# peteroh23/ModulationDetectionCNN

Measured on AMD Instinct MI355X. Metric: I/Q frames/sec (2x128, VT-CNN2, batch=2^20), higher is better.
Workload: dtype bf16; 1 GPU; vtcnn2-c11-bf16-n2^20; topology=vtcnn2, classes=11, frames_per_gpu=1048576, global_batch=1048576, parallelism=batch-shard x1 (no collective), outputs=softmax probabilities f32 + argmax int32, frames_per_forward_call=1048576, full=False

## Files before the change

### modulationdetectioncnn_amd/csrc/mdc_internal.h

```cpp
#pragma once
#include <hip/hip_runtime.h>
#include <cstdarg>
#include <cstdint>
#include <cstdio>
#include <exception>
#include <mutex>
#include <new>
#include <string>
#include <type_traits>
#include <vector>

#include "mdc.h"

namespace mdc {

void set_error(const char* fmt, ...);

template <class Fn>
inline int guarded(const char* what, Fn&& fn) noexcept {
    try {
        return fn();
    } catch (const std::bad_alloc&) {
        set_error("%s: out of host memory", what);
        return MDC_ENOMEM;
// ... 17 lines not shown

constexpr int kRows = 2;
constexpr int kSamples = 128;
constexpr int kFrameFloats = kRows * kSamples;

constexpr int kC1 = 256;
constexpr int kW1 = 130;
constexpr int kC2 = 80;
constexpr int kW2 = 132;
constexpr int kFeat = kC2 * kW2;
constexpr int kHid = 256;

__host__ __device__ constexpr int feat16_index(int w, int o) {
    return (w >> 1) * (2 * kC2) + (o < 64 ? (w & 1) * 64 + o : 128 + 2 * (o - 64) + (w & 1));
}

__host__ __device__ constexpr int feat8_index(int w, int o) {
    return (w >> 2) * (4 * kC2) + (o < 64 ? ((w >> 1) & 1) * 128 + 8 * (o >> 2) + 4 * (w & 1) + (o & 3) : 256 + 4 * (o - 64) + (w & 3));
}

__device__ __forceinline__ uint2 load8_unaligned(const unsigned char* p) {
    uint2 r;
    __builtin_memcpy(&r, p, 8);
    return r;
}

struct NfArgs {
    unsigned char* flags;
    unsigned long long* count;
    int poison;
// ... 148 lines not shown
```

### modulationdetectioncnn_amd/csrc/vtcnn2.hip

```cpp
#include "dense_chain_common.h"

#include <algorithm>
#include <cmath>

namespace mdc {

namespace {

__device__ __forceinline__ void glds16(const void* g, void* lds_wave_base) {
    const unsigned l = (unsigned)(size_t)(__attribute__((address_space(3))) unsigned char*)lds_wave_base;
    asm volatile("global_load_lds_dwordx4 %0, off" ::"v"(g), "{m0}"(l) : "memory");
}
__device__ __forceinline__ void glds_drain_and_barrier() {
    asm volatile("s_waitcnt vmcnt(0)" ::: "memory");
    __syncthreads();
}

constexpr int kChunk = 16;
constexpr int kNChunk = kC1 / kChunk;
constexpr int kWChunkFloats = 2 * 3 * 5 * 4 * 64;
constexpr int kXld = 133;
constexpr int kXinFloats = 4 * 2 * 16 * kXld;
constexpr size_t kConvF32Lds = (2 * kWChunkFloats + kXinFloats) * sizeof(float);

// ... 345 lines not shown
#pragma unroll
    for (int r = 0; r < 4; ++r) {
        const long row = row0 + fq * 4 + r;
        if (row < n) hid[row * kHid + col] = fmaxf(acc[r] + bias, 0.f);
    }
}

template <typename T>
__global__ void vt_unpermute_kernel(const T* __restrict__ feat, long n, float* __restrict__ out, float unscale) {
    const long i = (long)blockIdx.x * blockDim.x + threadIdx.x;
    if (i >= n * kFeat) return;
    const long f = i / kFeat;
    const int r = (int)(i % kFeat);
    const int o = r / kW2, w = r % kW2;
    if constexpr (sizeof(T) == 2) {
        const T v = feat[f * kFeat + feat16_index(w, o)];
        out[i] = __uint_as_float(((unsigned)v) << 16) * unscale;
    } else {
        out[i] = feat[(f * kW2 + w) * kC2 + o];
    }
}

__global__ void vt_unpermute8_kernel(const unsigned char* __restrict__ feat, long n, float* __restrict__ out, float unscale) {
    const long i = (long)blockIdx.x * blockDim.x + threadIdx.x;
    if (i >= n * kFeat) return;
    const long f = i / kFeat;
    const int r = (int)(i % kFeat);
    const int o = r / kW2, w = r % kW2;
    const unsigned v = feat[f * kFeat + feat8_index(w, o)];
    const int e = (int)((v >> 3) & 15u), mant = (int)(v & 7u);
    float mag = e == 0 ? ldexpf((float)mant, -9) : ldexpf(1.f + (float)mant * 0.125f, e - 7);
// ... 181 lines not shown
```

### modulationdetectioncnn_amd/csrc/vtcnn2_bf16.hip

```cpp
#include "vtcnn2_bf16_common.h"
#include "vtcnn2_sched_common.h"

#include <cmath>

#include <cstdlib>
#include <cstring>
#include <type_traits>

namespace mdc {

namespace {

#ifdef MDC_ALTERNATES
__global__ __launch_bounds__(256, 1) void vt_conv_bf16_kernel(const float* __restrict__ x, long n,
                                                              const u32x4* __restrict__ wq,
                                                              const u32x2* __restrict__ a1q,
                                                              const float* __restrict__ b2,
                                                              unsigned short* __restrict__ feat) {
    extern __shared__ __attribute__((aligned(16))) unsigned char smem[];
    unsigned* img = reinterpret_cast<unsigned*>(smem);
    float* part = reinterpret_cast<float*>(smem + (size_t)2 * kImgWords * 4);
    const int tid = threadIdx.x, lane = tid & 63;
    const int q = __builtin_amdgcn_readfirstlane(tid >> 6);
    const int nl = lane & 15, g = lane >> 4;
// ... 18 lines not shown

    for (int i = tid; i < 2 * kImgWords; i += 256) img[i] = ((i & 63) >= 48) ? 0x3F803F80u : 0u;
    __syncthreads();

    const long ngroups = (n + 15) >> 4;
    long grp = blockIdx.x;
    if (grp < ngroups)
        for (int k = 0; k < 4; ++k) stage_quarter(k, x, n, grp * 16, img, tid);
    __syncthreads();

    int buf = 0;
    for (; grp < ngroups; grp += gridDim.x, buf ^= 1) {
        const unsigned* im = img + buf * kImgWords + lane;
        const long frame0 = grp * 16;
        const long fme = frame0 + nl;
        unsigned short* fbase = feat + fme * (long)(kW2 * kC2) + 4 * g;
        const long gnext = grp + gridDim.x;

        f32x4 acc[3][5];
#pragma unroll
        for (int a = 0; a < 3; ++a)
#pragma unroll
            for (int b = 0; b < 5; ++b) acc[a][b] = f32x4{0.f, 0.f, 0.f, 0.f};
        bf16x8 Bf[2][2][2];
        f32x4 X[4][2];
        f32x4 rp[4];
        float rc[4];
        using I0 = std::integral_constant<int, 0>;
        using I1 = std::integral_constant<int, 1>;
        using I2 = std::integral_constant<int, 2>;

// ... 50 lines not shown
            const float* pw = part + PB * kPartFloats;
#pragma unroll
            for (int k = 0; k < 4; ++k) {
                rp[k] = *reinterpret_cast<const f32x4*>(pw + ((k * 5 + q) * 64 + lane) * 4);
                rc[k] = pw[((k * 5 + 4) * 64 + lane) * 4 + q];
            }
        };
        auto red_finish = [&](int w) {
            const f32x4 s = (rp[0] + rp[1]) + (rp[2] + rp[3]);
            u32x2 o;
            const f32x4 bq = *reinterpret_cast<const f32x4*>(bq_lds);
            o[0] = pack2relu(s[0] + bq[0], s[1] + bq[1]);
            o[1] = pack2relu(s[2] + bq[2], s[3] + bq[3]);
            const float t = ((rc[0] + rc[1]) + (rc[2] + rc[3])) + *b4_lds;
            const unsigned short t16 = (unsigned short)pack2relu(t, 0.f);
            unsigned short* frow = fbase - 4 * g;
            *reinterpret_cast<u32x2*>(frow + feat16_index(w, 16 * q + 4 * g)) = o;
            frow[feat16_index(w, 64 + 4 * g + q)] = t16;
        };
#define MDC_SB() __builtin_amdgcn_sched_barrier(0)
        auto step = [&](int v, auto par_next, auto first_tag, auto last_tag, f32x4 (&a0)[5], f32x4 (&a1)[5], f32x4 (&a2)[5]) {
            constexpr bool FIRST = decltype(first_tag)::value != 0, LAST = decltype(last_tag)::value != 0;
            using PB = std::integral_constant<int, 1 - decltype(par_next)::value>;
            if (!FIRST) { x_fence(I1{}); pack(PB{}, I1{}, I0{}); pack(PB{}, I1{}, I1{}); }
            if (!LAST) conv1_load(v + 1, par_next, I0{});
            tap(PB{}, I2{}, I0{}, I0{}, a2, false); tap(PB{}, I2{}, I0{}, I1{}, a2, false);
            tap(PB{}, I2{}, I1{}, I0{}, a2, false); tap(PB{}, I2{}, I1{}, I1{}, a2, false);
            part_write(PB{}, a2);
            if (!LAST) { conv1(par_next, I0{}); conv1_load(v + 1, par_next, I1{}); }
            tap(PB{}, I1{}, I0{}, I0{}, a1, false); tap(PB{}, I1{}, I0{}, I1{}, a1, false);
            tap(PB{}, I1{}, I1{}, I0{}, a1, false);
            if (!LAST) { x_fence(I0{}); pack(par_next, I0{}, I0{}); pack(par_next, I0{}, I1{}); }
            tap(PB{}, I1{}, I1{}, I1{}, a1, false);
// ... 129 lines not shown
```

### modulationdetectioncnn_amd/csrc/vtcnn2_bf16_dense1.hip

```cpp
#include "vtcnn2_bf16_common.h"
#include "dense_chain_common.h"

#include <cstdlib>

namespace mdc {

namespace {

constexpr int kBM = 256, kBN = 256, kBK = 64;
constexpr int kTileBytes = kBM * kBK * 2;
constexpr size_t kDenseBf16Lds = (size_t)4 * kTileBytes;
constexpr size_t kDenseHeadLds = (size_t)128 * kChainXld * 4;
static_assert(kDenseHeadLds >= kDenseBf16Lds, "the fused-head form allocates the larger of the two");
constexpr int kNT = kFeat / kBK;

__device__ __forceinline__ bf16x8 cvt_e4m3x8(u32x2 r) {
    const bf16x2 p0 = __builtin_amdgcn_cvt_scalef32_pk_bf16_fp8(r[0], 1.0f, false);
    const bf16x2 p1 = __builtin_amdgcn_cvt_scalef32_pk_bf16_fp8(r[0], 1.0f, true);
    const bf16x2 p2 = __builtin_amdgcn_cvt_scalef32_pk_bf16_fp8(r[1], 1.0f, false);
    const bf16x2 p3 = __builtin_amdgcn_cvt_scalef32_pk_bf16_fp8(r[1], 1.0f, true);
    return bf16x8{p0[0], p0[1], p1[0], p1[1], p2[0], p2[1], p3[0], p3[1]};
}


#if defined(MDC_ALTERNATES) || defined(MDC_ABLATIONS)
template <int ABL>
__global__ __launch_bounds__(512) void vt_dense1_bf16_kernel(const unsigned short* __restrict__ feat, long n,
                                                             const unsigned short* __restrict__ w1t,
                                                             const float* __restrict__ c1,
// ... 1 lines not shown
    extern __shared__ __attribute__((aligned(16))) unsigned char smem[];
    const int tid = threadIdx.x, lane = tid & 63;
    const int wv = __builtin_amdgcn_readfirstlane(tid >> 6);
    const int wr = wv >> 2, wc = wv & 3;
    const int fr = lane & 15, fg = lane >> 4;
    const long row0 = (long)blockIdx.x * kBM;

    const int srow = lane >> 3, spos = lane & 7;
    const unsigned short* asrc[4];
    const unsigned short* bsrc[4];
#pragma unroll
    for (int p = 0; p < 4; ++p) {
        const int r = (wv * 4 + p) * 8 + srow;
        long gr = (ABL == 1 ? 0 : row0) + r;
        if (gr >= n) gr = n - 1;
        asrc[p] = feat + gr * (long)kFeat + ((spos ^ (r & 7)) * 8);
        bsrc[p] = w1t + r * kBK + ((spos ^ (r & 7)) * 8);
    }
    auto stage = [&](int t, int b) {
        if (ABL == 3 && t > 1) return;
        unsigned char* A = smem + (size_t)b * 2 * kTileBytes;
        unsigned char* B = A + kTileBytes;
#pragma unroll
        for (int p = 0; p < 4; ++p) {
            glds16(asrc[p] + t * kBK, A + (wv * 4 + p) * 1024);
            glds16(bsrc[p] + (long)t * (kBN * kBK), B + (wv * 4 + p) * 1024);
        }
    };

    f32x4 acc[8][4];
#pragma unroll
    for (int i = 0; i < 8; ++i)
#pragma unroll
        for (int j = 0; j < 4; ++j) acc[i][j] = f32x4{0.f, 0.f, 0.f, 0.f};

    auto compute = [&](int b) {
        const unsigned char* A = smem + (size_t)b * 2 * kTileBytes;
        const unsigned char* B = A + kTileBytes;
#pragma unroll
        for (int ks = 0; ks < 2; ++ks) {
// ... 114 lines not shown
    const int wr = wv >> 2, wc = wv & 3;
    const int fr = lane & 15, fg = lane >> 4;
    const long row0 = (long)blockIdx.x * kBM;

    const int srow = lane >> 3, spos = lane & 7;
    const unsigned short* src[4][2];
#pragma unroll
    for (int j = 0; j < 2; ++j) {
        const int u = (wv * 2 + j) * 8 + srow;
        const int sw = (spos ^ (u & 7)) * 8;
        const int arow_lo = 128 * (u >> 6) + (u & 63);
        const int brow_lo = 64 * (u >> 5) + (u & 31);
        long g0 = (ABL == 1 ? 0 : row0) + arow_lo, g3 = (ABL == 1 ? 0 : row0) + arow_lo + 64;
        if (g0 >= n) g0 = n - 1;
        if (g3 >= n) g3 = n - 1;
        src[0][j] = feat + g0 * (long)kFeat + sw;
        src[3][j] = feat + g3 * (long)kFeat + sw;
        src[1][j] = w1t + brow_lo * kBK + sw;
        src[2][j] = w1t + (brow_lo + 32) * kBK + sw;
    }
    const unsigned char* src8[2] = {nullptr, nullptr};
    if constexpr (F8) {
        const int u = wv * 16 + (lane >> 2);
        const int sw = ((lane & 3) ^ ((u >> 2) & 3)) * 16;
        const int arow_lo = 128 * (u >> 6) + (u & 63);
        long g0 = row0 + arow_lo, g3 = row0 + arow_lo + 64;
        if (g0 >= n) g0 = n - 1;
        if (g3 >= n) g3 = n - 1;
        const unsigned char* f8 = reinterpret_cast<const unsigned char*>(feat);
        src8[0] = f8 + g0 * (long)kFeat + sw;
        src8[1] = f8 + g3 * (long)kFeat + sw;
    }
    auto stage_unit = [&](int t, int unit, int b) {
        if (ABL == 2 && (unit == 1 || unit == 2) && (t & 1)) return;
        unsigned char* dst = smem + ((size_t)b * 4 + unit) * kUnitBytes + (wv * 2) * 1024;
        if constexpr (F8) {
            if (unit == 0 || unit == 3) {
                glds16(src8[unit == 3] + (long)t * kBK, smem + ((size_t)b * 4 + unit) * kUnitBytes + wv * 1024);
                return;
            }
        }
        if (unit == 0 || unit == 3) {
            glds16_nt(src[unit][0] + (long)t * kBK, dst);
            glds16_nt(src[unit][1] + (long)t * kBK, dst + 1024);
        } else {
            glds16(src[unit][0] + (long)t * (kBN * kBK), dst);
            glds16(src[unit][1] + (long)t * (kBN * kBK), dst + 1024);
        }
    };

    auto frag = [&](const unsigned char* unit_base, int u, int ks) {
        return *reinterpret_cast<const bf16x8*>(unit_base + u * 128 + (((ks * 4 + fg) ^ (u & 7)) * 16));
    };

    f32x4 acc[8][4];
#pragma unroll
    for (int i = 0; i < 8; ++i)
#pragma unroll
        for (int j = 0; j < 4; ++j) acc[i][j] = f32x4{0.f, 0.f, 0.f, 0.f};
// ... 138 lines not shown

    d1_epilogue<HEAD>(acc, smem, row0, n, lane, wv, c1, hid, w2pack, n_out, probs, labels);
}


template <bool F8>
__global__ __launch_bounds__(64) void vt_dense1_bf16_small_kernel(const unsigned short* __restrict__ feat, long n,
                                                                  const unsigned short* __restrict__ w1t,
                                                                  const float* __restrict__ c1, float* __restrict__ hid) {
    const int lane = threadIdx.x, fr = lane & 15, fg = lane >> 4;
    const long row0 = (long)blockIdx.x * 16;
    const int col0 = blockIdx.y * 16;
    long ar = row0 + fr;
    if (ar >= n) ar = n - 1;
    using AFrag = typename std::conditional<F8, u32x2, bf16x8>::type;
    const unsigned char* ap = reinterpret_cast<const unsigned char*>(feat) + (ar * (long)kFeat + fg * 8) * (F8 ? 1 : 2);
    const unsigned short* bp = w1t + (long)(col0 + fr) * kBK + fg * 8;
    f32x4 acc = f32x4{0.f, 0.f, 0.f, 0.f};
    constexpr int kU = 5, kBlocks = kNT / kU;
    static_assert(kNT % kU == 0 && kBlocks % 2 == 1, "blocks: an even count in the loop, the last one drained after it");
    AFrag a0[kU][2], a1[kU][2];
    bf16x8 b0[kU][2], b1[kU][2];
    auto load = [&](AFrag (&af)[kU][2], bf16x8 (&bfr)[kU][2], int blk) {
#pragma unroll
        for (int u = 0; u < kU; ++u)
#pragma unroll
            for (int ks = 0; ks < 2; ++ks) {
                af[u][ks] = *reinterpret_cast<const AFrag*>(ap + ((blk * kU + u) * kBK + ks * 32) * (F8 ? 1 : 2));
                bfr[u][ks] = *reinterpret_cast<const bf16x8*>(bp + (long)(blk * kU + u) * (kBN * kBK) + ks * 32);
            }
    };
    auto mma = [&](const AFrag (&af)[kU][2], const bf16x8 (&bfr)[kU][2]) {
#pragma unroll
        for (int u = 0; u < kU; ++u)
#pragma unroll
            for (int ks = 0; ks < 2; ++ks) {
                bf16x8 a;
                if constexpr (F8) a = cvt_e4m3x8(af[u][ks]); else a = af[u][ks];
                acc = __builtin_amdgcn_mfma_f32_16x16x32_bf16(a, bfr[u][ks], acc, 0, 0, 0);
            }
    };
    load(a0, b0, 0);
    for (int blk = 0; blk < kBlocks - 1; blk += 2) {
// ... 19 lines not shown
template <bool F8>
__global__ __launch_bounds__(256) void vt_dense1_bf16_coop_kernel(const unsigned short* __restrict__ feat, long n,
                                                                  const unsigned short* __restrict__ w1t,
                                                                  const float* __restrict__ c1, float* __restrict__ hid) {
    extern __shared__ __attribute__((aligned(16))) unsigned char smem[];
    const int tid = threadIdx.x, lane = tid & 63, fr = lane & 15, fg = lane >> 4;
    const int wv = __builtin_amdgcn_readfirstlane(tid >> 6);
    const long row0 = (long)blockIdx.x * 16;
    const int col0 = blockIdx.y * 16;
    long ar = row0 + fr;
    if (ar >= n) ar = n - 1;
    const unsigned char* src;
    long kstep;
    if (wv < 2) {
        if constexpr (F8) { src = reinterpret_cast<const unsigned char*>(feat) + ar * (long)kFeat + fg * 16; kstep = kBK; }
        else { src = reinterpret_cast<const unsigned char*>(feat + ar * (long)kFeat + fg * 8 + (wv & 1) * 32); kstep = 2L * kBK; }
    } else {
        src = reinterpret_cast<const unsigned char*>(w1t + (long)(col0 + fr) * kBK + fg * 8 + (wv & 1) * 32);
        kstep = 2L * kBN * kBK;
    }
    const bool copies = !(F8 && wv == 1);
    static_assert(kRing % kGrp == 0, "groups do not straddle the ring's end");
    constexpr int kAhead = kRing / kGrp - 1;
    constexpr int kGroups = kNT / kGrp, kTail = kNT - kGroups * kGrp;
    auto issue = [&](int g) {
#pragma unroll
        for (int j = 0; j < kGrp; ++j) {
            const int t = g * kGrp + j, tc = t < kNT ? t : kNT - 1;
            if (copies) glds16_async(src + tc * kstep, smem + (size_t)(t % kRing) * 4096 + wv * 1024);
        }
    };
// ... 144 lines not shown
```

### modulationdetectioncnn_amd/csrc/vtcnn2_bf16_sched.hip

```cpp
#include "vtcnn2_bf16_common.h"
#include "vtcnn2_sched_common.h"

#include <cmath>
#include <cstdlib>
#include <type_traits>

namespace mdc {

namespace {

constexpr int kNV = 24;

struct SchedState {
    u32x4 Wv[kNV];
    u32x4 Wa[kWFrags - kNV];
    f32x4 bias[5];
    u32x4 A1[2];
    unsigned Bf[2][2][2][4];
    f32x16 X[2];
    f32x4 rp[4];
    float rc[4];
    float tprev;
    u32x4 L0[3];
    u32x4 L1;
// ... 14 lines not shown
        static_assert(IDX >= kNV, "padded form written for the AGPR-resident fragments only");
        asm volatile("s_nop 1\n\tv_mfma_f32_16x16x32_bf16 %0, %1, %2, %0" : "+a"(acc[OT]) : "a"(st.Wa[IDX - kNV]), "v"(b));
    } else {
        if constexpr (IDX < kNV) asm volatile("v_mfma_f32_16x16x32_bf16 %0, %1, %2, %0" : "+a"(acc[OT]) : "v"(st.Wv[IDX]), "v"(b));
        else asm volatile("v_mfma_f32_16x16x32_bf16 %0, %1, %2, %0" : "+a"(acc[OT]) : "a"(st.Wa[IDX - kNV]), "v"(b));
    }
}
template <int SP, int U>
__device__ __forceinline__ void sch_packop(SchedState& st) {
    constexpr int CT = U >> 3, j = U & 7;
    unsigned& d = st.Bf[SP][CT][j >> 2][j & 3];
    const float lo = st.X[CT][2 * j], hi = st.X[CT][2 * j + 1];
    asm volatile("v_cvt_pk_bf16_f32 %0, %1, %2 clamp" : "=v"(d) : "v"(lo), "v"(hi));
}
template <int V12, bool FIRST, bool LAST, int ABL, bool RANGE = false>
__device__ __forceinline__ void sch_step(SchedState& st, int v, int q, unsigned short* fbase, f32x4 (&acc)[3][5], int wlo = 0) {
    constexpr int PAR = V12 & 1, PN = 1 - PAR;
    constexpr int R1 = (V12 + 1) & 3, S0 = ((V12 + 1) >> 2) % 3, SN = (S0 + 1) % 3;
    constexpr bool kLoadEven = (V12 & 3) == 1 && !LAST, kLoadOdd = (V12 & 3) == 3 && !LAST;
    constexpr int LSLOT = ((V12 >> 2) + 1) % 3;
    constexpr bool kExch = ABL != 2 && ABL != 6, kFin = ABL != 3 && ABL != 6, kC1 = ABL != 5 && ABL != 6;
    f32x4 (&a2)[5] = acc[V12 % 3];
    f32x4 (&a1)[5] = acc[(V12 + 1) % 3];
    f32x4 (&a0)[5] = acc[(V12 + 2) % 3];
    const unsigned load_addr = st.im_addr + ((v >> 2) * 16 + (kLoadEven ? 16 : 24));
    FinTmp ft;
    FinOut fo;
    constexpr int OP = (V12 + 1) & 1;
#define FIN(K) do { if (!FIRST && kFin) sch_fin_clamp<K, OP>(st, ft, fo); } while (0)
#define PREP(I) do { if (!LAST && kC1 && ABL != 11) sch_prep<R1, S0, SN, I>(st); } while (0)
#define C1M(CT) do { if (!LAST && kC1) sch_conv1_mfma<R1, S0, CT>(st); } while (0)
#define ST(W) do { if (!FIRST && kFin && (W == 0 || OP == 1)) { if (ABL == 7) { if (W == 0) asm volatile("" ::"v"(fo.o0), "v"(fo.o1)); else asm volatile("" ::"v"(fo.tt)); } else if (!RANGE || v - 1 >= wlo) sch_store<W>(fo, fbase, v - 1, q, st.gs); } } while (0)
#define WR(OT) do { if (kExch && ABL != 8) sch_part_write<PAR, OT>(st, a2[OT]); } while (0)
#define PK(N) do { if (!LAST && kC1 && ABL != 10) sch_packop<PN, N>(st); } while (0)
#define RD(R) do { if (kExch && ABL != 9) sch_red_load1<PAR, R>(st); } while (0)
#define LD() do { if (kC1 && ABL != 11) { if (kLoadEven) sch_load_even<LSLOT>(st, load_addr); else if (kLoadOdd) sch_load_odd(st, load_addr); } } while (0)
#ifdef MDC_F8_PROBE_HALF_BARRIER
    constexpr bool kHalfBarrierSkip = (V12 & 1) == 1;
#else
    constexpr bool kHalfBarrierSkip = false;
#endif
#define HANDOFF() do { \
        if (ABL == 1 || kHalfBarrierSkip) asm volatile("s_waitcnt lgkmcnt(0)" ::: "memory"); \
        else if (kExch) asm volatile("s_waitcnt lgkmcnt(0)\n\ts_barrier" ::: "memory"); \
        asm volatile("" ::"a"(a2[0]), "a"(a2[1]), "a"(a2[2]), "a"(a2[3]), "a"(a2[4])); } while (0)
    sch_wait_lds(st);
    sch_tap<PAR, 2, 0, RANGE && (V12 == 1 || V12 == 2)>(st, a2); FIN(0);
// ... 47 lines not shown
    sch_tap<PAR, 0, 6>(st, a0); HANDOFF();
    sch_tap<PAR, 0, 7>(st, a0); RD(0);
    sch_tap<PAR, 0, 8>(st, a0); RD(1);
    sch_tap<PAR, 0, 9>(st, a0); RD(2);
    sch_tap<PAR, 0, 10>(st, a0); RD(3);
    sch_tap<PAR, 0, 11>(st, a0); RD(4);
    sch_tap<PAR, 0, 12>(st, a0); RD(5);
    sch_tap<PAR, 0, 13>(st, a0); RD(6);
    sch_tap<PAR, 0, 14>(st, a0); RD(7);
    sch_tap<PAR, 0, 15>(st, a0); LD();
    sch_tap<PAR, 0, 16>(st, a0);
    sch_tap<PAR, 0, 17>(st, a0);
    sch_tap<PAR, 0, 18>(st, a0);
    sch_tap<PAR, 0, 19>(st, a0);
    if (ABL == 10 && !LAST) asm volatile("" ::"v"(st.X[0]), "v"(st.X[1]));
#undef FIN
#undef PREP
#undef C1M
#undef ST
#undef WR
#undef PK
#undef RD
#undef LD
#undef HANDOFF
}

template <int ABL, bool U8 = false, bool RANGE = false>
__global__ __launch_bounds__(256, 1) void vt_conv_bf16_sched_kernel(const float* __restrict__ x, long n,
                                                                    const u32x4* __restrict__ wq, const u32x4* __restrict__ a1q,
                                                                    const float* __restrict__ b2, unsigned short* __restrict__ feat,
// ... 37 lines not shown

    for (int i = tid; i < 2 * kSImgWords; i += 256) img[i] = ((((i / kS) & 63) >= 32) && ((i % kS) & 1)) ? 0x3F803F80u : 0u;
    __syncthreads();
    const long ngroups = (n + 15) >> 4;
    long grp = blockIdx.x;
    if (grp < ngroups)
        for (int k = 0; k < 4; ++k) sch_stage_write(k, stage_decode<U8>(stage_load<U8>(k, x, n, grp * 16, tid, hop2), tid, scale), n, grp * 16, img, tid);
    __syncthreads();
    const int rng = RANGE ? (int)blockIdx.y : 0;
    const int S = 12 * rng;
    const int wlo = rng ? S + 2 : 0;

    int buf = 0;
    for (; grp < ngroups; grp += gridDim.x, buf ^= 1) {
        st.im_addr = img_lds + (buf * kSImgWords + lane * kS) * 4;
        unsigned short* fbase = feat + (grp * 16 + fs) * (long)(kW2 * kC2);
        const long gnext = RANGE ? ngroups : grp + gridDim.x;
        f32x4 acc[3][5];
        {
            const u32x4 zero = u32x4{0u, 0u, 0u, 0u};
#pragma unroll
            for (int b = 0; b < 5; ++b) {
                asm volatile("s_nop 1\n\tv_mfma_f32_16x16x32_bf16 %0, %1, %1, %2" : "=&a"(acc[0][b]) : "v"(zero), "a"(st.bias[b]));
                asm volatile("v_mfma_f32_16x16x32_bf16 %0, %1, %1, %2" : "=&a"(acc[1][b]) : "v"(zero), "a"(st.bias[b]));
            }
        }

        sch_load_even<0>(st, st.im_addr + (S >> 2) * 16);
        sch_load_odd(st, st.im_addr + (S >> 2) * 16 + 8);
        sch_wait_lds(st);
        sch_conv1_mfma<0, 0, 0>(st); sch_conv1_mfma<0, 0, 1>(st);
        asm volatile("s_nop 7\n\ts_nop 7\n\ts_nop 7\n\ts_nop 7\n\ts_nop 7\n\ts_nop 7\n\ts_nop 7\n\ts_nop 7" : "+v"(st.X[0]), "+v"(st.X[1]));
        [&]<int... N>(std::integer_sequence<int, N...>) { (sch_packop<0, N>(st), ...); }(std::make_integer_sequence<int, 16>{});
        asm volatile("s_nop 1");

        sch_step<0, true, false, ABL, RANGE>(st, S, q, fbase, acc, wlo);
        const int iters = RANGE ? (rng < 10 ? 1 : 0) : 10;
        int v = S + 1;
        typename StageRaw<U8>::type sv{};
        for (int it = 0; it < iters; ++it, v += 12) {
            if constexpr (!RANGE) {
                if (it >= 6 && gnext < ngroups) sch_stage_write(it - 6, stage_decode<U8>(sv, tid, scale), n, gnext * 16, img + (buf ^ 1) * kSImgWords, tid);
                if (it >= 5 && it < 9 && gnext < ngroups) sv = stage_load<U8>(it - 5, x, n, gnext * 16, tid, hop2);
            }
            sch_step<1, false, false, ABL, RANGE>(st, v + 0, q, fbase, acc, wlo);
            sch_step<2, false, false, ABL, RANGE>(st, v + 1, q, fbase, acc, wlo);
            sch_step<3, false, false, ABL, RANGE>(st, v + 2, q, fbase, acc, wlo);
            sch_step<4, false, false, ABL, RANGE>(st, v + 3, q, fbase, acc, wlo);
            sch_step<5, false, false, ABL, RANGE>(st, v + 4, q, fbase, acc, wlo);
            sch_step<6, false, false, ABL, RANGE>(st, v + 5, q, fbase, acc, wlo);
            sch_step<7, false, false, ABL, RANGE>(st, v + 6, q, fbase, acc, wlo);
            sch_step<8, false, false, ABL, RANGE>(st, v + 7, q, fbase, acc, wlo);
            sch_step<9, false, false, ABL, RANGE>(st, v + 8, q, fbase, acc, wlo);
            sch_step<10, false, false, ABL, RANGE>(st, v + 9, q, fbase, acc, wlo);
            sch_step<11, false, false, ABL, RANGE>(st, v + 10, q, fbase, acc, wlo);
            sch_step<0, false, false, ABL, RANGE>(st, v + 11, q, fbase, acc, wlo);
        }
        const int vt = RANGE ? v : 121;
        sch_step<1, false, false, ABL, RANGE>(st, vt, q, fbase, acc, wlo);
        if constexpr (RANGE) {
            if (rng < 10) {
                FinOut fo;
                sch_wait_lds(st);
                sch_fin_all_clamp<1>(st, fo);
                sch_store<0>(fo, fbase, vt, q, st.gs);
                sch_store<1>(fo, fbase, vt, q, st.gs);
                asm volatile("s_nop 7\n\ts_nop 7" ::"a"(acc[0][0]), "a"(acc[1][0]), "a"(acc[2][0]));
                __syncthreads();
                continue;
            }
        }
        sch_step<2, false, false, ABL, RANGE>(st, 122, q, fbase, acc, wlo);
        sch_step<3, false, false, ABL, RANGE>(st, 123, q, fbase, acc, wlo);
        sch_step<4, false, false, ABL, RANGE>(st, 124, q, fbase, acc, wlo);
        sch_step<5, false, false, ABL, RANGE>(st, 125, q, fbase, acc, wlo);
        sch_step<6, false, false, ABL, RANGE>(st, 126, q, fbase, acc, wlo);
        sch_step<7, false, false, ABL, RANGE>(st, 127, q, fbase, acc, wlo);
        sch_step<8, false, false, ABL, RANGE>(st, 128, q, fbase, acc, wlo);
        sch_step<9, false, true, ABL, RANGE>(st, 129, q, fbase, acc, wlo);
        auto finish_store = [&](auto odd, int w) {
            FinOut fo;
            sch_wait_lds(st);
            sch_fin_all_clamp<decltype(odd)::value>(st, fo);
            sch_store<0>(fo, fbase, w, q, st.gs);
            if constexpr (decltype(odd)::value) sch_store<1>(fo, fbase, w, q, st.gs);
        };
        using Even = std::integral_constant<int, 0>;
        using Odd = std::integral_constant<int, 1>;
        finish_store(Odd{}, 129);
        asm volatile("s_nop 7\n\ts_nop 7");
        sch_part_write<0, 0>(st, acc[1][0]); sch_part_write<0, 1>(st, acc[1][1]); sch_part_write<0, 2>(st, acc[1][2]);
        sch_part_write<0, 3>(st, acc[1][3]); sch_part_write<0, 4>(st, acc[1][4]);
        asm volatile("s_waitcnt lgkmcnt(0)\n\ts_barrier" ::: "memory");
        sch_red_load<0>(st);
        asm volatile("" ::"a"(acc[1][0]), "a"(acc[1][1]), "a"(acc[1][2]), "a"(acc[1][3]), "a"(acc[1][4]));
        finish_store(Even{}, 130);
        sch_part_write<1, 0>(st, acc[2][0]); sch_part_write<1, 1>(st, acc[2][1]); sch_part_write<1, 2>(st, acc[2][2]);
        sch_part_write<1, 3>(st, acc[2][3]); sch_part_write<1, 4>(st, acc[2][4]);
        asm volatile("s_waitcnt lgkmcnt(0)\n\ts_barrier" ::: "memory");
        sch_red_load<1>(st);
        asm volatile("" ::"a"(acc[2][0]), "a"(acc[2][1]), "a"(acc[2][2]), "a"(acc[2][3]), "a"(acc[2][4]));
        finish_store(Odd{}, 131);
        __syncthreads();
    }
}

}

int vtcnn2_bf16_pack_sched(mdc_model* m) {
    const float* k1 = m->hk[0].data();
    const float* b1 = m->hb[0].data();
    const float* k2 = m->hk[1].data();
    int rc;
    std::vector<unsigned short> wq((size_t)4 * kWFrags * 64 * 8);
    for (int q = 0; q < 4; ++q)
        for (int ct = 0; ct < 2; ++ct)
            for (int j = 0; j < 3; ++j)
// ... 68 lines not shown
```

### modulationdetectioncnn_amd/csrc/vtcnn2_fp8_conv.hip

```cpp
#include "vtcnn2_bf16_common.h"
#include "vtcnn2_sched_common.h"

#include <cmath>
#include <cstdlib>

namespace mdc {

namespace {

using u32x8 = __attribute__((ext_vector_type(8))) unsigned;
constexpr int kF8Frags = 15;
constexpr int kF8NV = 7;

struct Fp8State {
    u32x8 Wv[kF8NV];
    u32x8 Wa[kF8Frags - kF8NV];
    f32x4 bias[5];
    u32x4 A1[2];
    unsigned Bf[2][8];
    unsigned one;
    unsigned scb;
    float sc9;
    f32x16 X[2];
    unsigned T[16];
// ... 200 lines not shown

    for (int i = tid; i < 2 * kSImgWords; i += 256) img[i] = ((((i / kS) & 63) >= 32) && ((i % kS) & 1)) ? 0x3F803F80u : 0u;
    __syncthreads();
    const long ngroups = (n + 15) >> 4;
    long grp = blockIdx.x;
    if (grp < ngroups)
        for (int k = 0; k < 4; ++k) sch_stage_write(k, stage_decode<U8>(stage_load<U8>(k, x, n, grp * 16, tid, hop2), tid, scale), n, grp * 16, img, tid);
    __syncthreads();
    const int rng = RANGE ? (int)blockIdx.y : 0;
    const int S = 12 * rng;
    const int wlo = rng ? S + 2 : 0;

    int buf = 0;
    for (; grp < ngroups; grp += gridDim.x, buf ^= 1) {
        st.im_addr = img_lds + (buf * kSImgWords + lane * kS) * 4;
        FeatT* fbase = feat + (grp * 16 + fs) * (long)(kW2 * kC2);
        const long gnext = RANGE ? ngroups : grp + gridDim.x;
        f32x4 acc[3][5];
        {
            const u32x4 zero = u32x4{0u, 0u, 0u, 0u};
#pragma unroll
            for (int b = 0; b < 5; ++b) {
                asm volatile("s_nop 1\n\tv_mfma_f32_16x16x32_bf16 %0, %1, %1, %2" : "=&a"(acc[0][b]) : "v"(zero), "a"(st.bias[b]));
                asm volatile("v_mfma_f32_16x16x32_bf16 %0, %1, %1, %2" : "=&a"(acc[1][b]) : "v"(zero), "a"(st.bias[b]));
            }
        }
        sch_load_even<0>(st, st.im_addr + (S >> 2) * 16);
        sch_load_odd(st, st.im_addr + (S >> 2) * 16 + 8);
        sch_wait_lds(st);
        sch_conv1_mfma<0, 0, 0>(st); sch_conv1_mfma<0, 0, 1>(st);
        asm volatile("s_nop 7\n\ts_nop 7\n\ts_nop 7\n\ts_nop 7\n\ts_nop 7\n\ts_nop 7\n\ts_nop 7\n\ts_nop 7" : "+v"(st.X[0]), "+v"(st.X[1]));
// ... 225 lines not shown
```

### modulationdetectioncnn_amd/csrc/vtcnn2_sched_common.h

```cpp
#pragma once
#include "vtcnn2_bf16_common.h"

#include <type_traits>
#include <utility>

namespace mdc {

namespace {

constexpr int kS = 140;
constexpr int kSImgWords = 64 * kS;
constexpr long kConvRangeFrames = 1024;
constexpr size_t kSchedLds = (size_t)2 * kSImgWords * 4 + (size_t)2 * kPartFloats * 4;

using f32x16 = __attribute__((ext_vector_type(16))) float;

template <int SLOT, class S>
__device__ __forceinline__ void sch_load_even(S& st, unsigned entry_addr) {
    asm volatile("ds_read_b128 %0, %1" : "=v"(st.L0[SLOT]) : "v"(entry_addr) : "memory");
}
template <class S>
__device__ __forceinline__ void sch_load_odd(S& st, unsigned entry_addr) {
    asm volatile("ds_read2_b64 %0, %1 offset0:0 offset1:1" : "=v"(st.L1) : "v"(entry_addr) : "memory");
}
// ... 51 lines not shown
    else if constexpr (K == 14) asm volatile("v_add_f32 %0, %1, %2" : "=v"(f.a) : "v"(st.rc[0]), "v"(st.rc[1]));
    else if constexpr (K == 15) asm volatile("v_add_f32 %0, %1, %2" : "=v"(f.b) : "v"(st.rc[2]), "v"(st.rc[3]));
    else if constexpr (K == 16) {
        if constexpr (ODD) asm volatile("v_add_f32 %0, %1, %2" : "=v"(f.t) : "v"(f.a), "v"(f.b));
        else asm volatile("v_add_f32 %0, %1, %2" : "=v"(st.tprev) : "v"(f.a), "v"(f.b));
    } else if constexpr (ODD) asm volatile("v_cvt_pk_bf16_f32 %0, %1, %2 clamp" : "=v"(out.tt) : "v"(st.tprev), "v"(f.t));
}
template <int ODD, class S>
__device__ __forceinline__ void sch_fin_all_clamp(S& st, FinOut& out) {
    FinTmp f;
    [&]<int... K>(std::integer_sequence<int, K...>) { (sch_fin_clamp<K, ODD>(st, f, out), ...); }(std::make_integer_sequence<int, 18>{});
}

template <int WHICH>
__device__ __forceinline__ void sch_store(const FinOut& fo, unsigned short* frow, int w, int q, int gs) {
    unsigned short* pair = frow + (long)(w >> 1) * (2 * kC2);
    if constexpr (WHICH == 0) *reinterpret_cast<u32x2*>(pair + (w & 1) * 64 + 16 * q + 4 * gs) = u32x2{fo.o0, fo.o1};
    else *reinterpret_cast<unsigned*>(pair + 128 + 2 * (4 * q + gs)) = fo.tt;
}

__device__ __forceinline__ void sch_stage_write(int k, float4 v, long n, long frame0, unsigned* __restrict__ im, int tid) {
    const int idx = tid + 256 * k;
    const int i = idx >> 6, l = idx & 63;
    if (frame0 + i >= n) v = make_float4(0.f, 0.f, 0.f, 0.f);
    const int h = l >> 5, m = l & 31;
    const float xs[4] = {v.x, v.y, v.z, v.w};
#pragma unroll
    for (int e = 0; e < 2; ++e) {
        const float a = xs[2 * e], b = xs[2 * e + 1];
        const unsigned hi = pack2(a, b);
        const float ah = __uint_as_float(hi << 16), bh = __uint_as_float(hi & 0xFFFF0000u);
        const unsigned lo = pack2(a - ah, b - bh);
        unsigned* d = im + (i + 16 * h) * kS + 2 * (2 * m + 1 + e);
// ... 10 lines not shown
```

Baseline: 41.34 million frames/s.

## Store bf16 conv features pre-tiled in dense GEMM A-tile layout

Changes the bf16 intermediate feature tensor from row-major per frame to a tiled layout of 256-row by 64-element K-chunks that matches the dense1 GEMM's A tiles. Each GEMM K-step then reads one contiguous tile instead of striding across frames. The conv kernels' stores now go through per-dozen scalar base addresses with global_store instructions. That may improve GEMM load locality and cut store address arithmetic, but the conv writes become more scattered across tiles. All producers and consumers, including unpermute and fallback paths, are updated to the new indexing.

```diff
diff --git a/modulationdetectioncnn_amd/csrc/mdc_internal.h b/modulationdetectioncnn_amd/csrc/mdc_internal.h
--- a/modulationdetectioncnn_amd/csrc/mdc_internal.h
+++ b/modulationdetectioncnn_amd/csrc/mdc_internal.h
@@ -55,6 +55,14 @@
 __host__ __device__ constexpr int feat16_index(int w, int o) {
     return (w >> 1) * (2 * kC2) + (o < 64 ? (w & 1) * 64 + o : 128 + 2 * (o - 64) + (w & 1));
 }
+
+constexpr int kFeatTileRows = 256, kFeatChunk = 64;
+constexpr long kFeatKTile = (long)kFeatTileRows * kFeatChunk;
+constexpr long kFeatTile = (long)(kFeat / kFeatChunk) * kFeatKTile;
+static_assert(kFeat % kFeatChunk == 0, "whole K-tiles");
+__host__ __device__ constexpr long feat16_row(long f) { return (f >> 8) * kFeatTile + (f & 255) * kFeatChunk; }
+__host__ __device__ constexpr long feat16_k(int kk) { return (long)(kk >> 6) * kFeatKTile + (kk & 63); }
+__host__ __device__ constexpr long feat16_offset(long f, int kk) { return feat16_row(f) + feat16_k(kk); }
 
 __host__ __device__ constexpr int feat8_index(int w, int o) {
     return (w >> 2) * (4 * kC2) + (o < 64 ? ((w >> 1) & 1) * 128 + 8 * (o >> 2) + 4 * (w & 1) + (o & 3) : 256 + 4 * (o - 64) + (w & 3));
diff --git a/modulationdetectioncnn_amd/csrc/vtcnn2.hip b/modulationdetectioncnn_amd/csrc/vtcnn2.hip
--- a/modulationdetectioncnn_amd/csrc/vtcnn2.hip
+++ b/modulationdetectioncnn_amd/csrc/vtcnn2.hip
@@ -383,7 +383,7 @@
     const int r = (int)(i % kFeat);
     const int o = r / kW2, w = r % kW2;
     if constexpr (sizeof(T) == 2) {
-        const T v = feat[f * kFeat + feat16_index(w, o)];
+        const T v = feat[feat16_offset(f, feat16_index(w, o))];
         out[i] = __uint_as_float(((unsigned)v) << 16) * unscale;
     } else {
         out[i] = feat[(f * kW2 + w) * kC2 + o];
diff --git a/modulationdetectioncnn_amd/csrc/vtcnn2_bf16.hip b/modulationdetectioncnn_amd/csrc/vtcnn2_bf16.hip
--- a/modulationdetectioncnn_amd/csrc/vtcnn2_bf16.hip
+++ b/modulationdetectioncnn_amd/csrc/vtcnn2_bf16.hip
@@ -56,7 +56,7 @@
         const unsigned* im = img + buf * kImgWords + lane;
         const long frame0 = grp * 16;
         const long fme = frame0 + nl;
-        unsigned short* fbase = feat + fme * (long)(kW2 * kC2) + 4 * g;
+        unsigned short* frow = feat + feat16_row(fme);
         const long gnext = grp + gridDim.x;
 
         f32x4 acc[3][5];
@@ -137,9 +137,8 @@
             o[1] = pack2relu(s[2] + bq[2], s[3] + bq[3]);
             const float t = ((rc[0] + rc[1]) + (rc[2] + rc[3])) + *b4_lds;
             const unsigned short t16 = (unsigned short)pack2relu(t, 0.f);
-            unsigned short* frow = fbase - 4 * g;
-            *reinterpret_cast<u32x2*>(frow + feat16_index(w, 16 * q + 4 * g)) = o;
-            frow[feat16_index(w, 64 + 4 * g + q)] = t16;
+            *reinterpret_cast<u32x2*>(frow + feat16_k(feat16_index(w, 16 * q + 4 * g))) = o;
+            frow[feat16_k(feat16_index(w, 64 + 4 * g + q))] = t16;
         };
 #define MDC_SB() __builtin_amdgcn_sched_barrier(0)
         auto step = [&](int v, auto par_next, auto first_tag, auto last_tag, f32x4 (&a0)[5], f32x4 (&a1)[5], f32x4 (&a2)[5]) {
diff --git a/modulationdetectioncnn_amd/csrc/vtcnn2_bf16_dense1.hip b/modulationdetectioncnn_amd/csrc/vtcnn2_bf16_dense1.hip
--- a/modulationdetectioncnn_amd/csrc/vtcnn2_bf16_dense1.hip
+++ b/modulationdetectioncnn_amd/csrc/vtcnn2_bf16_dense1.hip
@@ -13,6 +13,7 @@
 constexpr size_t kDenseHeadLds = (size_t)128 * kChainXld * 4;
 static_assert(kDenseHeadLds >= kDenseBf16Lds, "the fused-head form allocates the larger of the two");
 constexpr int kNT = kFeat / kBK;
+static_assert(kBM == kFeatTileRows && kBK == kFeatChunk, "the bf16 feature tensor is stored in this GEMM's A tiles (feat16_offset)");
 
 __device__ __forceinline__ bf16x8 cvt_e4m3x8(u32x2 r) {
     const bf16x2 p0 = __builtin_amdgcn_cvt_scalef32_pk_bf16_fp8(r[0], 1.0f, false);
@@ -44,7 +45,7 @@
         const int r = (wv * 4 + p) * 8 + srow;
         long gr = (ABL == 1 ? 0 : row0) + r;
         if (gr >= n) gr = n - 1;
-        asrc[p] = feat + gr * (long)kFeat + ((spos ^ (r & 7)) * 8);
+        asrc[p] = feat + feat16_row(gr) + ((spos ^ (r & 7)) * 8);
         bsrc[p] = w1t + r * kBK + ((spos ^ (r & 7)) * 8);
     }
     auto stage = [&](int t, int b) {
@@ -53,7 +54,7 @@
         unsigned char* B = A + kTileBytes;
 #pragma unroll
         for (int p = 0; p < 4; ++p) {
-            glds16(asrc[p] + t * kBK, A + (wv * 4 + p) * 1024);
+            glds16(asrc[p] + t * kFeatKTile, A + (wv * 4 + p) * 1024);
             glds16(bsrc[p] + (long)t * (kBN * kBK), B + (wv * 4 + p) * 1024);
         }
     };
@@ -198,8 +199,8 @@
         long g0 = (ABL == 1 ? 0 : row0) + arow_lo, g3 = (ABL == 1 ? 0 : row0) + arow_lo + 64;
         if (g0 >= n) g0 = n - 1;
         if (g3 >= n) g3 = n - 1;
-        src[0][j] = feat + g0 * (long)kFeat + sw;
-        src[3][j] = feat + g3 * (long)kFeat + sw;
+        src[0][j] = feat + feat16_row(g0) + sw;
+        src[3][j] = feat + feat16_row(g3) + sw;
         src[1][j] = w1t + brow_lo * kBK + sw;
         src[2][j] = w1t + (brow_lo + 32) * kBK + sw;
     }
@@ -225,8 +226,8 @@
             }
         }
         if (unit == 0 || unit == 3) {
-            glds16_nt(src[unit][0] + (long)t * kBK, dst);
-            glds16_nt(src[unit][1] + (long)t * kBK, dst + 1024);
+            glds16_nt(src[unit][0] + (long)t * kFeatKTile, dst);
+            glds16_nt(src[unit][1] + (long)t * kFeatKTile, dst + 1024);
         } else {
             glds16(src[unit][0] + (long)t * (kBN * kBK), dst);
             glds16(src[unit][1] + (long)t * (kBN * kBK), dst + 1024);
@@ -395,7 +396,8 @@
     long ar = row0 + fr;
     if (ar >= n) ar = n - 1;
     using AFrag = typename std::conditional<F8, u32x2, bf16x8>::type;
-    const unsigned char* ap = reinterpret_cast<const unsigned char*>(feat) + (ar * (long)kFeat + fg * 8) * (F8 ? 1 : 2);
+    const unsigned char* ap = reinterpret_cast<const unsigned char*>(feat) + (F8 ? ar * (long)kFeat + fg * 8 : (feat16_row(ar) + fg * 8) * 2);
+    constexpr long kAStep = F8 ? kBK : 2 * kFeatKTile;
     const unsigned short* bp = w1t + (long)(col0 + fr) * kBK + fg * 8;
     f32x4 acc = f32x4{0.f, 0.f, 0.f, 0.f};
     constexpr int kU = 5, kBlocks = kNT / kU;
@@ -407,7 +409,7 @@
         for (int u = 0; u < kU; ++u)
 #pragma unroll
             for (int ks = 0; ks < 2; ++ks) {
-                af[u][ks] = *reinterpret_cast<const AFrag*>(ap + ((blk * kU + u) * kBK + ks * 32) * (F8 ? 1 : 2));
+                af[u][ks] = *reinterpret_cast<const AFrag*>(ap + (blk * kU + u) * kAStep + ks * (F8 ? 32 : 64));
                 bfr[u][ks] = *reinterpret_cast<const bf16x8*>(bp + (long)(blk * kU + u) * (kBN * kBK) + ks * 32);
             }
     };
@@ -457,7 +459,7 @@
     long kstep;
     if (wv < 2) {
         if constexpr (F8) { src = reinterpret_cast<const unsigned char*>(feat) + ar * (long)kFeat + fg * 16; kstep = kBK; }
-        else { src = reinterpret_cast<const unsigned char*>(feat + ar * (long)kFeat + fg * 8 + (wv & 1) * 32); kstep = 2L * kBK; }
+        else { src = reinterpret_cast<const unsigned char*>(feat + feat16_row(ar) + fg * 8 + (wv & 1) * 32); kstep = 2L * kFeatKTile; }
     } else {
         src = reinterpret_cast<const unsigned char*>(w1t + (long)(col0 + fr) * kBK + fg * 8 + (wv & 1) * 32);
         kstep = 2L * kBN * kBK;
diff --git a/modulationdetectioncnn_amd/csrc/vtcnn2_bf16_sched.hip b/modulationdetectioncnn_amd/csrc/vtcnn2_bf16_sched.hip
--- a/modulationdetectioncnn_amd/csrc/vtcnn2_bf16_sched.hip
+++ b/modulationdetectioncnn_amd/csrc/vtcnn2_bf16_sched.hip
@@ -52,7 +52,7 @@
     asm volatile("v_cvt_pk_bf16_f32 %0, %1, %2 clamp" : "=v"(d) : "v"(lo), "v"(hi));
 }
 template <int V12, bool FIRST, bool LAST, int ABL, bool RANGE = false>
-__device__ __forceinline__ void sch_step(SchedState& st, int v, int q, unsigned short* fbase, f32x4 (&acc)[3][5], int wlo = 0) {
+__device__ __forceinline__ void sch_step(SchedState& st, int v, SchFeatAddr& fa, f32x4 (&acc)[3][5], int wlo = 0) {
     constexpr int PAR = V12 & 1, PN = 1 - PAR;
     constexpr int R1 = (V12 + 1) & 3, S0 = ((V12 + 1) >> 2) % 3, SN = (S0 + 1) % 3;
     constexpr bool kLoadEven = (V12 & 3) == 1 && !LAST, kLoadOdd = (V12 & 3) == 3 && !LAST;
@@ -68,7 +68,7 @@
 #define FIN(K) do { if (!FIRST && kFin) sch_fin_clamp<K, OP>(st, ft, fo); } while (0)
 #define PREP(I) do { if (!LAST && kC1 && ABL != 11) sch_prep<R1, S0, SN, I>(st); } while (0)
 #define C1M(CT) do { if (!LAST && kC1) sch_conv1_mfma<R1, S0, CT>(st); } while (0)
-#define ST(W) do { if (!FIRST && kFin && (W == 0 || OP == 1)) { if (ABL == 7) { if (W == 0) asm volatile("" ::"v"(fo.o0), "v"(fo.o1)); else asm volatile("" ::"v"(fo.tt)); } else if (!RANGE || v - 1 >= wlo) sch_store<W>(fo, fbase, v - 1, q, st.gs); } } while (0)
+#define ST(W) do { if (!FIRST && kFin && (W == 0 || OP == 1)) { if (ABL == 7) { if (W == 0) asm volatile("" ::"v"(fo.o0), "v"(fo.o1)); else asm volatile("" ::"v"(fo.tt)); } else if (!RANGE || v - 1 >= wlo) sch_store_dozen<W, (V12 + 11) % 12>(fo, fa); } } while (0)
 #define WR(OT) do { if (kExch && ABL != 8) sch_part_write<PAR, OT>(st, a2[OT]); } while (0)
 #define PK(N) do { if (!LAST && kC1 && ABL != 10) sch_packop<PN, N>(st); } while (0)
 #define RD(R) do { if (kExch && ABL != 9) sch_red_load1<PAR, R>(st); } while (0)
@@ -146,6 +146,7 @@
     sch_tap<PAR, 0, 18>(st, a0);
     sch_tap<PAR, 0, 19>(st, a0);
     if (ABL == 10 && !LAST) asm volatile("" ::"v"(st.X[0]), "v"(st.X[1]));
+    if constexpr (V12 == 0 && !FIRST) sch_feat_next_dozen(fa);
 #undef FIN
 #undef PREP
 #undef C1M
@@ -213,7 +214,8 @@
     int buf = 0;
     for (; grp < ngroups; grp += gridDim.x, buf ^= 1) {
         st.im_addr = img_lds + (buf * kSImgWords + lane * kS) * 4;
-        unsigned short* fbase = feat + (grp * 16 + fs) * (long)(kW2 * kC2);
+        SchFeatAddr fa;
+        sch_feat_group(fa, feat, grp, q, fs, gs, rng);
         const long gnext = RANGE ? ngroups : grp + gridDim.x;
         f32x4 acc[3][5];
         {
@@ -233,7 +235,7 @@
         [&]<int... N>(std::integer_sequence<int, N...>) { (sch_packop<0, N>(st), ...); }(std::make_integer_sequence<int, 16>{});
         asm volatile("s_nop 1");
 
-        sch_step<0, true, false, ABL, RANGE>(st, S, q, fbase, acc, wlo);
+        sch_step<0, true, false, ABL, RANGE>(st, S, fa, acc, wlo);
         const int iters = RANGE ? (rng < 10 ? 1 : 0) : 10;
         int v = S + 1;
         typename StageRaw<U8>::type sv{};
@@ -242,64 +244,63 @@
                 if (it >= 6 && gnext < ngroups) sch_stage_write(it - 6, stage_decode<U8>(sv, tid, scale), n, gnext * 16, img + (buf ^ 1) * kSImgWords, tid);
                 if (it >= 5 && it < 9 && gnext < ngroups) sv = stage_load<U8>(it - 5, x, n, gnext * 16, tid, hop2);
             }
-            sch_step<1, false, false, ABL, RANGE>(st, v + 0, q, fbase, acc, wlo);
-            sch_step<2, false, false, ABL, RANGE>(st, v + 1, q, fbase, acc, wlo);
-            sch_step<3, false, false, ABL, RANGE>(st, v + 2, q, fbase, acc, wlo);
-            sch_step<4, false, false, ABL, RANGE>(st, v + 3, q, fbase, acc, wlo);
-            sch_step<5, false, false, ABL, RANGE>(st, v + 4, q, fbase, acc, wlo);
-            sch_step<6, false, false, ABL, RANGE>(st, v + 5, q, fbase, acc, wlo);
-            sch_step<7, false, false, ABL, RANGE>(st, v + 6, q, fbase, acc, wlo);
-            sch_step<8, false, false, ABL, RANGE>(st, v + 7, q, fbase, acc, wlo);
-            sch_step<9, false, false, ABL, RANGE>(st, v + 8, q, fbase, acc, wlo);
-            sch_step<10, false, false, ABL, RANGE>(st, v + 9, q, fbase, acc, wlo);
-            sch_step<11, false, false, ABL, RANGE>(st, v + 10, q, fbase, acc, wlo);
-            sch_step<0, false, false, ABL, RANGE>(st, v + 11, q, fbase, acc, wlo);
+            sch_step<1, false, false, ABL, RANGE>(st, v + 0, fa, acc, wlo);
+            sch_step<2, false, false, ABL, RANGE>(st, v + 1, fa, acc, wlo);
+            sch_step<3, false, false, ABL, RANGE>(st, v + 2, fa, acc, wlo);
+            sch_step<4, false, false, ABL, RANGE>(st, v + 3, fa, acc, wlo);
+            sch_step<5, false, false, ABL, RANGE>(st, v + 4, fa, acc, wlo);
+            sch_step<6, false, false, ABL, RANGE>(st, v + 5, fa, acc, wlo);
+            sch_step<7, false, false, ABL, RANGE>(st, v + 6, fa, acc, wlo);
+            sch_step<8, false, false, ABL, RANGE>(st, v + 7, fa, acc, wlo);
+            sch_step<9, false, false, ABL, RANGE>(st, v + 8, fa, acc, wlo);
+            sch_step<10, false, false, ABL, RANGE>(st, v + 9, fa, acc, wlo);
+            sch_step<11, false, false, ABL, RANGE>(st, v + 10, fa, acc, wlo);
+            sch_step<0, false, false, ABL, RANGE>(st, v + 11, fa, acc, wlo);
         }
         const int vt = RANGE ? v : 121;
-        sch_step<1, false, false, ABL, RANGE>(st, vt, q, fbase, acc, wlo);
+        sch_step<1, false, false, ABL, RANGE>(st, vt, fa, acc, wlo);
         if constexpr (RANGE) {
             if (rng < 10) {
                 FinOut fo;
                 sch_wait_lds(st);
                 sch_fin_all_clamp<1>(st, fo);
-                sch_store<0>(fo, fbase, vt, q, st.gs);
-                sch_store<1>(fo, fbase, vt, q, st.gs);
+                sch_store_dozen<0, 1>(fo, fa);
+                sch_store_dozen<1, 1>(fo, fa);
                 asm volatile("s_nop 7\n\ts_nop 7" ::"a"(acc[0][0]), "a"(acc[1][0]), "a"(acc[2][0]));
                 __syncthreads();
                 continue;
             }
         }
-        sch_step<2, false, false, ABL, RANGE>(st, 122, q, fbase, acc, wlo);
-        sch_step<3, false, false, ABL, RANGE>(st, 123, q, fbase, acc, wlo);
-        sch_step<4, false, false, ABL, RANGE>(st, 124, q, fbase, acc, wlo);
-        sch_step<5, false, false, ABL, RANGE>(st, 125, q, fbase, acc, wlo);
-        sch_step<6, false, false, ABL, RANGE>(st, 126, q, fbase, acc, wlo);
-        sch_step<7, false, false, ABL, RANGE>(st, 127, q, fbase, acc, wlo);
-        sch_step<8, false, false, ABL, RANGE>(st, 128, q, fbase, acc, wlo);
-        sch_step<9, false, true, ABL, RANGE>(st, 129, q, fbase, acc, wlo);
-        auto finish_store = [&](auto odd, int w) {
+        sch_step<2, false, false, ABL, RANGE>(st, 122, fa, acc, wlo);
+        sch_step<3, false, false, ABL, RANGE>(st, 123, fa, acc, wlo);
+        sch_step<4, false, false, ABL, RANGE>(st, 124, fa, acc, wlo);
+        sch_step<5, false, false, ABL, RANGE>(st, 125, fa, acc, wlo);
+        sch_step<6, false, false, ABL, RANGE>(st, 126, fa, acc, wlo);
+        sch_step<7, false, false, ABL, RANGE>(st, 127, fa, acc, wlo);
+        sch_step<8, false, false, ABL, RANGE>(st, 128, fa, acc, wlo);
+        sch_step<9, false, true, ABL, RANGE>(st, 129, fa, acc, wlo);
+        auto finish_store = [&](auto w_tag) {
+            constexpr int W12 = decltype(w_tag)::value % 12, ODD = W12 & 1;
             FinOut fo;
             sch_wait_lds(st);
-            sch_fin_all_clamp<decltype(odd)::value>(st, fo);
-            sch_store<0>(fo, fbase, w, q, st.gs);
-            if constexpr (decltype(odd)::value) sch_store<1>(fo, fbase, w, q, st.gs);
+            sch_fin_all_clamp<ODD>(st, fo);
+            sch_store_dozen<0, W12>(fo, fa);
+            if constexpr (ODD) sch_store_dozen<1, W12>(fo, fa);
         };
-        using Even = std::integral_constant<int, 0>;
-        using Odd = std::integral_constant<int, 1>;
-        finish_store(Odd{}, 129);
+        finish_store(std::integral_constant<int, 129>{});
         asm volatile("s_nop 7\n\ts_nop 7");
         sch_part_write<0, 0>(st, acc[1][0]); sch_part_write<0, 1>(st, acc[1][1]); sch_part_write<0, 2>(st, acc[1][2]);
         sch_part_write<0, 3>(st, acc[1][3]); sch_part_write<0, 4>(st, acc[1][4]);
         asm volatile("s_waitcnt lgkmcnt(0)\n\ts_barrier" ::: "memory");
         sch_red_load<0>(st);
         asm volatile("" ::"a"(acc[1][0]), "a"(acc[1][1]), "a"(acc[1][2]), "a"(acc[1][3]), "a"(acc[1][4]));
-        finish_store(Even{}, 130);
+        finish_store(std::integral_constant<int, 130>{});
         sch_part_write<1, 0>(st, acc[2][0]); sch_part_write<1, 1>(st, acc[2][1]); sch_part_write<1, 2>(st, acc[2][2]);
         sch_part_write<1, 3>(st, acc[2][3]); sch_part_write<1, 4>(st, acc[2][4]);
         asm volatile("s_waitcnt lgkmcnt(0)\n\ts_barrier" ::: "memory");
         sch_red_load<1>(st);
         asm volatile("" ::"a"(acc[2][0]), "a"(acc[2][1]), "a"(acc[2][2]), "a"(acc[2][3]), "a"(acc[2][4]));
-        finish_store(Odd{}, 131);
+        finish_store(std::integral_constant<int, 131>{});
         __syncthreads();
     }
 }
diff --git a/modulationdetectioncnn_amd/csrc/vtcnn2_fp8_conv.hip b/modulationdetectioncnn_amd/csrc/vtcnn2_fp8_conv.hip
--- a/modulationdetectioncnn_amd/csrc/vtcnn2_fp8_conv.hip
+++ b/modulationdetectioncnn_amd/csrc/vtcnn2_fp8_conv.hip
@@ -238,7 +238,7 @@
     int buf = 0;
     for (; grp < ngroups; grp += gridDim.x, buf ^= 1) {
         st.im_addr = img_lds + (buf * kSImgWords + lane * kS) * 4;
-        FeatT* fbase = feat + (grp * 16 + fs) * (long)(kW2 * kC2);
+        FeatT* fbase = feat + (F8OUT ? (grp * 16 + fs) * (long)(kW2 * kC2) : feat16_row(grp * 16 + fs));
         const long gnext = RANGE ? ngroups : grp + gridDim.x;
         f32x4 acc[3][5];
         {
diff --git a/modulationdetectioncnn_amd/csrc/vtcnn2_sched_common.h b/modulationdetectioncnn_amd/csrc/vtcnn2_sched_common.h
--- a/modulationdetectioncnn_amd/csrc/vtcnn2_sched_common.h
+++ b/modulationdetectioncnn_amd/csrc/vtcnn2_sched_common.h
@@ -89,9 +89,43 @@
 
 template <int WHICH>
 __device__ __forceinline__ void sch_store(const FinOut& fo, unsigned short* frow, int w, int q, int gs) {
-    unsigned short* pair = frow + (long)(w >> 1) * (2 * kC2);
-    if constexpr (WHICH == 0) *reinterpret_cast<u32x2*>(pair + (w & 1) * 64 + 16 * q + 4 * gs) = u32x2{fo.o0, fo.o1};
-    else *reinterpret_cast<unsigned*>(pair + 128 + 2 * (4 * q + gs)) = fo.tt;
+    const int pair = (w >> 1) * (2 * kC2);
+    if constexpr (WHICH == 0) *reinterpret_cast<u32x2*>(frow + feat16_k(pair + (w & 1) * 64 + 16 * q) + 4 * gs) = u32x2{fo.o0, fo.o1};
+    else *reinterpret_cast<unsigned*>(frow + feat16_k(pair + 128 + 8 * q) + 2 * gs) = fo.tt;
+}
+
+struct SchFeatAddr {
+    unsigned char* base[2];
+    unsigned char* tail;
+    unsigned lane_main, lane_tail;
+};
+constexpr long kSchDozenBytes = 15 * kFeatKTile * 2;
+static_assert(12 / 2 * 2 * kC2 == 15 * kFeatChunk, "a dozen positions is a whole number of K-tiles");
+__device__ __forceinline__ void sch_feat_group(SchFeatAddr& a, unsigned short* feat, long grp, int q, int fs, int gs, int dozen) {
+    unsigned char* g = reinterpret_cast<unsigned char*>(feat + feat16_row(grp * 16)) + dozen * kSchDozenBytes;
+    a.base[0] = g + feat16_k(16 * q) * 2;
+    a.base[1] = g + feat16_k(32 + 16 * q) * 2;
+    a.tail = g + 8 * q * 2;
+    a.lane_main = (unsigned)(fs * kFeatChunk * 2 + gs * 8);
+    a.lane_tail = (unsigned)(fs * kFeatChunk * 2 + gs * 4);
+}
+__device__ __forceinline__ void sch_feat_next_dozen(SchFeatAddr& a) {
+    a.base[0] += kSchDozenBytes; a.base[1] += kSchDozenBytes; a.tail += kSchDozenBytes;
+}
+template <int WHICH, int W12>
+__device__ __forceinline__ void sch_store_dozen(const FinOut& fo, const SchFeatAddr& a) {
+    constexpr int P = W12 >> 1, PAR = P & 1;
+    if constexpr (WHICH == 0) {
+        constexpr int kc = 160 * P + 64 * (W12 & 1) - 32 * PAR;
+        static_assert(kc % 64 == 0 && kc >= 0, "the pair's start without its half K-tile");
+        unsigned char* sb = a.base[PAR] + (kc / 64) * kFeatKTile * 2;
+        asm volatile("global_store_dwordx2 %0, %1, %2" ::"v"(a.lane_main), "v"(u32x2{fo.o0, fo.o1}), "s"(sb) : "memory");
+    } else {
+        constexpr int kc = 160 * P + 128;
+        static_assert((kc & 63) == 32 * PAR, "the tail segment starts 0 or 32 elements into its chunk");
+        unsigned char* sb = a.tail + feat16_k(kc) * 2;
+        asm volatile("global_store_dword %0, %1, %2" ::"v"(a.lane_tail), "v"(fo.tt), "s"(sb) : "memory");
+    }
 }
 
 __device__ __forceinline__ void sch_stage_write(int k, float4 v, long n, long frame0, unsigned* __restrict__ im, int tid) {
```

New measurement: 41.57 million frames/s (median of 6 runs). Within noise of the previous version (+0.5%).
